# ryanelandt/PressureFieldContact.jl

Hardware: AMD Instinct MI355X
Metric: tet-tri clip+integrate ops/s (higher is better)
Workload: dtype f64

## Files before the change

pressurefieldcontact.jl_amd/csrc/pfc_hip.hip:

```cpp
#include "pfc_kernels.h"

#include <atomic>
#include <condition_variable>
#include <functional>
#include <mutex>
#include <thread>
#include <cmath>
#include <cstdlib>
#include <limits>
#include <cstdarg>
#include <cstdio>
#include <cstring>
#include <string>
#include <vector>

#include "../../include/pfc.h"
#include "pfc_sort.h"

namespace pfc {

__global__ void k_prep_tri(int n, const double *__restrict__ pt, const int *__restrict__ tri, TriRec *__restrict__ out) {
    int k = blockIdx.x * blockDim.x + threadIdx.x;
    if (k >= n) return;
    V3 a = ld3(pt + 3 * tri[3 * k]), b = ld3(pt + 3 * tri[3 * k + 1]), c = ld3(pt + 3 * tri[3 * k + 2]);
// ... 350 lines not shown
        hints[0].n = n; hints[0].sparse = sparse;
    }
    bool shape_is_sparse(int n) const {
        for (const ShapeHint &e : hints) if (e.n == n) return e.sparse;
        return false;
    }
    long long last_tslots = 0;
    Event ev[EV_COUNT];
    bool ev_valid = false;
    pfc_context *twin = nullptr;
    bool is_twin = false;
    DevBuf<int> fout;
    PinBuf<int> h_fout;
    int *fout_dev = nullptr;
    const int *fout_host = nullptr;
    int opt_fused = 1;
    int opt_fixed_order = 0;
    DevBuf<int> det;
    DevBuf<unsigned long long> sort_keys[2];
    DevBuf<int> canon_off, canon_fill, canon_item;
    int sort_tmp_items = 0;
    bool fixed_whole_list = false;
    DevBuf<char> sort_tmp;
    size_t sort_tmp_for = 0;
    int sort_tmp_bits = 0;
    int max_elem1 = 1, max_elem2 = 1;
    DevBuf<double> fx_rec, vfx_rec;
    DevBuf<int> vfx_head;
    DevBuf<int> fx_head;
    long long surv_sorted_serial = -1;
    size_t sort_cover = 0;
    size_t sort_cover_used = 0;
    int opt_vertex_fields = 1;
    int opt_clip_queue = 1;
    int fused_skip = 0;
    int fused_seq = 0;
    int fu_nw = 1;
    int last_fu_nw = 0, last_team = 0;
    int n_cu = 0;
    int opt_team = 48;
    DevBuf<unsigned long long> team;
    DevBuf<int> emit_ctr;
    PinBuf<int> h_emit;
    PinBuf<unsigned> h_more;
    bool fu_emit = false;
    int dual_fused_skip = 0;
    const double *fu_dpose = nullptr, *fu_dtwist = nullptr;
    double *fu_dwrench = nullptr, *fu_dsdot = nullptr;
    int fu_ndir = 0;
    bool pending_fused = false, last_fused = false;
    int opt_split_min = 1025;
    int opt_clip_min = 384;
    int opt_poison = 0;
    int split_n0 = 0;
    bool in_split = false;
    int last_parts = 1;
    Event ev_fork, ev_join, ev_join0;
    int twin_queue_fallback = 0;
    DevBuf<long long> surf_cnt, surf_off, surf_out;
    DevBuf<double> surf_part;
    DevBuf<int> surf_seg, surf_canon_off, surf_canon_fill, surf_canon_item;
    DevBuf<double> ljac_seed;
    DevBuf<double> ljac_out;
    DevBuf<double> ljac_io;
    DevBuf<int> ljac_ids;
    DevBuf<unsigned long long> surf_keys[2];
// ... 161 lines not shown
    double *d = h->trac_d.p;
    t.item = h->trac_item.p;
    t.nx = d; t.ny = d + n; t.nz = d + 2 * n; t.rx = d + 3 * n; t.ry = d + 4 * n; t.rz = d + 5 * n;
    t.dA = d + 6 * n; t.p = d + 7 * n;
    return t;
}

int eff_levels(const pfc_context *h) {
    return (h->opt_max_levels > 0 && h->opt_max_levels < h->max_levels) ? h->opt_max_levels : h->max_levels;
}

constexpr int kDualSelectMin = 512;
constexpr int kBpSmallBlockMin = 3072;

int bfs_levels_for(const pfc_context *h, int n_items, int levels) {
    int L = 0;
    if (h->opt_bfs_levels >= 0) {
        L = h->opt_bfs_levels;
    } else {
        const bool big = h->max_leaves >= 8192, mid = h->max_leaves >= 1024;
        const int n_eff = h->in_split ? 2 * n_items : n_items;
        const double target = big ? (n_eff >= 600 ? 1.0 : (n_eff >= 256 ? 1024.0 : (n_eff >= 128 ? 2048.0 : (n_eff >= 32 ? 16384.0 : 49152.0))))
                                  : (mid ? 256.0 : 64.0);
        double seeds = (double)n_items;
        while (seeds < target && L < 9) { seeds *= 4.0; ++L; }
    }
    return L > levels ? levels : L;
}

bool pile_mode(const pfc_context *h, int n_items) {
    return h->max_leaves < 8192 && n_items >= 1024 && n_items < kBpSmallBlockMin && h->shape_is_sparse(n_items) && !h->is_twin;
}

int bp_block_for(const pfc_context *h, int n_items) {
    if (n_items >= kBpSmallBlockMin) return 128;
    if (h->in_split) return 256;
    if (h->max_leaves >= 8192 && n_items >= 8 && n_items < 1024) return 512;
    if (pile_mode(h, n_items)) return 512;
    return 256;
}

void launch_broadphase(pfc_context *h, int n_items, int L, int *ccount, int *fcount, int *next_seed, int *ucount, hipStream_t st) {
    for (int lv = 0; lv < L; ++lv) {
        BpArgs b;
        b.items = h->items.p; b.fin = h->frontier[lv & 1].p; b.fout = h->frontier[(lv + 1) & 1].p;
        b.cand = h->cand.p; b.fcount = fcount; b.ccount = ccount; b.icnt = h->icnt.p; b.status = h->status.p;
        b.level = lv; b.fcap = (int)h->fcap; b.ccap = (int)h->ccap; b.n_items = n_items;
        double ub = (double)n_items * std::pow(4.0, (double)(lv < 15 ? lv : 15));
        size_t bound = ub > (double)h->fcap ? h->fcap : (size_t)ub;
        hipLaunchKernelGGL(k_bp_expand, dim3(grid_for(bound, 256, 2048)), dim3(256), 0, st, b);
    }
    {
        double ub = (double)n_items * std::pow(4.0, (double)(L < 15 ? L : 15));
        size_t bound = ub > (double)h->fcap ? h->fcap : (size_t)ub;
        DfsArgs d;
        d.items = h->items.p; d.cand = h->cand.p; d.ccount = ccount; d.ccap = (int)h->ccap; d.icnt = h->icnt.p;
        d.status = h->status.p; d.reserve = 3 * h->max_levels + 3; d.stamps = h->stamps.p; d.n_items = n_items;
        if (h->opt_no_filter) {
            d.seeds = h->frontier[L & 1].p; d.n_seed = fcount + L; d.seed_cap = (int)h->fcap; d.next_seed = next_seed;
            d.no_filter = 1;
            hipLaunchKernelGGL(k_bp_dfs, dim3(grid_for(bound, 1, 256 * 8)), dim3(64), 0, st, d);
        } else {
            Dfs32Args f;
            f.items = h->items.p; f.seeds = h->frontier[L & 1].p; f.n_seed = fcount + L; f.next_seed = next_seed;
            f.seed_cap = (int)h->fcap; f.cand = h->cand.p; f.ccount = ccount; f.ccap = (int)h->ccap;
            f.ucount = ucount; f.icnt = h->icnt.p; f.status = h->status.p; f.stamps = h->stamps.p;
// ... 57 lines not shown
    NpArgs np;
    np.items = h->items.p; np.cand = h->cand.p; np.ccount = ccount; np.ccap = (int)h->ccap; np.acc = h->acc.p;
    np.icnt = h->icnt.p; np.n_items = n_items; np.clip_n = h->opt_debug ? h->clip_n.p : nullptr; np.trac = trac_view(h);
    np.tcount = tcount; np.tcap = (int)h->tcap; np.status = h->status.p; np.debug = h->opt_debug;
    np.stamps = h->stamps.p;
    np.rec = h->rec.p; np.rgn = h->rgn.p; np.rr_cap = (int)(h->rcap / kRgn);
    np.poly_item = h->poly_item.p; np.poly = h->poly.p; np.pcap = (int)poly_cap(h->ccap);
    np.pcnt = h->pcnt.p; np.chunk_switch = kNpChunkSwitch; np.poly_cand = h->want_surv ? h->poly_cand.p : nullptr;
    np.surv = h->want_surv ? h->surv.p : nullptr; np.scount = pcount + 1;
    const int np_grid = grid_for(h->ccap, kNpBlock, kNpMaxBlocks);
    const int np_mode = h->opt_debug ? 1 : ((h->opt_fixed_order || (h->opt_clip_min > 0 && n_items >= h->opt_clip_min)) ? 2 : 0);
    if (np_mode == 1) {
        if (h->any_tet_tet) hipLaunchKernelGGL((k_narrow<true, 1>), dim3(np_grid), dim3(kNpBlock), 0, st, np);
        else hipLaunchKernelGGL((k_narrow<false, 1>), dim3(np_grid), dim3(kNpBlock), 0, st, np);
    } else if (np_mode == 0) {
        if (h->any_tet_tet) hipLaunchKernelGGL((k_narrow<true, 0>), dim3(np_grid), dim3(kNpBlock), 0, st, np);
        else hipLaunchKernelGGL((k_narrow<false, 0>), dim3(np_grid), dim3(kNpBlock), 0, st, np);
    } else {
        if (h->opt_clip_queue && !h->any_tet_tet) {
            hipLaunchKernelGGL(k_clip_queue, dim3(np_grid), dim3(kNpBlock), 0, st, np);
        } else if (h->in_split || (n_items >= 640 && n_items < 1024)) {
            if (h->any_tet_tet) hipLaunchKernelGGL((k_narrow<true, 3>), dim3(np_grid), dim3(kNpBlock), 0, st, np);
            else hipLaunchKernelGGL((k_narrow<false, 3>), dim3(np_grid), dim3(kNpBlock), 0, st, np);
        } else {
            if (h->any_tet_tet) hipLaunchKernelGGL((k_narrow<true, 2>), dim3(np_grid), dim3(kNpBlock), 0, st, np);
            else hipLaunchKernelGGL((k_narrow<false, 2>), dim3(np_grid), dim3(kNpBlock), 0, st, np);
        }
        IntegArgs ig;
        ig.items = h->items.p; ig.n_items = n_items; ig.ccount = ccount; ig.ccap = (int)h->ccap; ig.chunk_switch = kNpChunkSwitch;
        ig.pcnt = h->pcnt.p; ig.poly_item = h->poly_item.p; ig.poly = h->poly.p; ig.pcap = np.pcap;
        ig.poly_cand = np.poly_cand; ig.surv = np.surv; ig.scount = np.scount; ig.acc = h->acc.p; ig.rec = h->rec.p;
        ig.rgn = h->rgn.p; ig.rr_cap = np.rr_cap; ig.icnt = h->icnt.p; ig.status = h->status.p;
        ig.det = h->opt_fixed_order ? h->det.p : nullptr;
        if (h->opt_fixed_order) hipLaunchKernelGGL(k_integ_fixed, dim3(grid_for(h->ccap, 64, kNpMaxBlocks)), dim3(64), 0, st, ig);
        else hipLaunchKernelGGL(k_integ, dim3(grid_for(h->ccap, 64, kNpMaxBlocks)), dim3(64), 0, st, ig);
    }
    if (prof) HIP_TRY(h, hipEventRecord(h->ev[EV_NP], st));

    BrArgs br;
    br.items = h->items.p; br.n_items = n_items; br.acc = h->acc.p; br.res = h->res.p; br.icnt = h->icnt.p;
    br.trac = trac_view(h); br.tcount = tcount; br.tcap = (int)h->tcap; br.wrench = d_wrench; br.sdot = d_sdot;
    br.counts = d_counts;
    br.ctr = h->ctr.p; br.n_ctr = levels + 12; br.status = h->status.p; br.tail = h->tail_dev ? h->tail_dev : h->tail.p;
    br.rgn = h->rgn.p; br.i_pcount = (levels + 9) & ~1;
    if (h->opt_fixed_order && np_mode == 2) {
        FixedArgs fx;
        fx.rec = h->rec.p; fx.det = h->det.p; fx.n_items = n_items; fx.n_slots = (int)(h->rcap / kRgn) * kRgn; fx.items = h->items.p;
        fx.acc = h->acc.p; fx.status = h->status.p;
        hipLaunchKernelGGL(k_shift_fixed, dim3(n_items), dim3(64), 0, st, fx);
    }
    if (h->any_bristle) {
        ShiftArgs sh;
        sh.rec = h->rec.p; sh.rgn = h->rgn.p; sh.rr_cap = (int)(h->rcap / kRgn); sh.acc = h->acc.p;
        if (!(h->opt_fixed_order && np_mode == 2)) hipLaunchKernelGGL(k_shift, dim3(grid_for(h->rcap, 64, 2048)), dim3(64), 0, st, sh);
        hipLaunchKernelGGL(k_eig, dim3(n_items), dim3(64), 0, st, br);
        FricArgs fr;
        fr.items = h->items.p; fr.poly_item = h->poly_item.p; fr.poly = h->poly.p; fr.ccount = ccount; fr.ccap = (int)h->ccap;
        fr.chunk_switch = kNpChunkSwitch; fr.pcnt = h->pcnt.p;
        fr.pcap = np.pcap; fr.res = h->res.p; fr.acc = h->acc.p;
        fr.n_items = n_items; fr.status = h->status.p;
        fr.sink = FixedSink{nullptr, nullptr, nullptr, 0, 0, 0, 0, 0, nullptr};
        if (h->opt_fixed_order && np_mode == 2) {
            const size_t n_pos = h->ccap / 64 + 1, cap = fixed_fric_cap(h->ccap, n_items);
            HIP_TRY(h, hipMemsetAsync(h->vfx_head.p, 0xFF, sizeof(int) * (size_t)n_items, st));
            HIP_TRY(h, hipMemsetAsync(h->vfx_head.p + n_items, 0, sizeof(int) * 2, st));
            fr.sink = FixedSink{h->vfx_rec.p, h->vfx_head.p + n_items, h->vfx_head.p, 0, 2, (int)n_pos, (int)(2 * n_pos), (int)cap, h->status.p};
        }
        const bool vertex_fields = h->opt_vertex_fields && !h->opt_debug;
// ... 752 lines not shown
    if (!h) return PFC_ERR_BAD_ARG;
    if (h->multi)
        return multi_eval_device(h, n_items, 0, d_ins_ids, d_pose, nullptr, d_twist, d_s, nullptr, nullptr, nullptr, d_wrench, d_sdot,
                                 nullptr, nullptr, d_counts, stream);
    { const int rc = check_eval_args(h, n_items, d_ins_ids, d_pose, d_twist, d_s, d_wrench, d_sdot); if (rc != PFC_OK) return rc; }
    if (n_items == 0) { h->pending = false; h->last_n_items = 0; return PFC_OK; }
    HIP_TRY(h, hipSetDevice(h->device));
    hipStream_t st = stream ? (hipStream_t)stream : h->stream;
    h->split_n0 = 0;
    h->pending_fused = false;
    end_kept_pass(h);
    h->pending_more = false;
    int team = fused_team(h, n_items);
    if (team > 1 && !team_acquire(h)) team = fused_ok(h, n_items) ? 1 : 0;
    if (team) {
        h->fu_nw = team;
        const int rc_t = enqueue_fused(h, n_items, d_ins_ids, d_pose, d_twist, d_s, d_wrench, d_sdot, d_counts, st);
        h->fu_nw = 1;
        if (rc_t != PFC_OK) team_release(h);
        return rc_t;
    }
    if (h->fused_skip > 0 && n_items <= kFusedMaxItems) --h->fused_skip;
    const bool split = h->opt_split_min > 0 && n_items >= h->opt_split_min && d_ins_ids && !h->opt_debug && !h->opt_fixed_order &&
                       !h->want_surv && !h->is_twin && !pile_mode(h, n_items);
    if (!split) return enqueue_eval(h, n_items, d_ins_ids, d_pose, d_twist, d_s, d_wrench, d_sdot, d_counts, st);
    int rc = make_twin(h);
    if (rc != PFC_OK) return rc;
    pfc_context *t = h->twin;
    t->opt_profile = h->opt_profile; t->opt_max_levels = h->opt_max_levels; t->opt_bfs_levels = h->opt_bfs_levels;
    t->opt_poison = h->opt_poison;
    if (t->opt_clip_min != h->opt_clip_min) { t->opt_clip_min = h->opt_clip_min; t->ghave[0] = t->ghave[1] = false; }
    if (t->opt_clip_queue != h->opt_clip_queue) { t->opt_clip_queue = h->opt_clip_queue; t->ghave[0] = t->ghave[1] = false; }
    if (t->opt_vertex_fields != h->opt_vertex_fields) { t->opt_vertex_fields = h->opt_vertex_fields; t->ghave[0] = t->ghave[1] = false; }
    t->opt_graph = h->opt_graph;
    if (t->opt_no_filter != h->opt_no_filter) { t->opt_no_filter = h->opt_no_filter; t->ghave[0] = t->ghave[1] = false; }
    const int n0 = n_items / 2, n1 = n_items - n0;
    hipStream_t s0 = h->stream;
    HIP_TRY(h, hipEventRecord(h->ev_fork, st));
    if (s0 != st) HIP_TRY(h, hipStreamWaitEvent(s0, h->ev_fork, 0));
    HIP_TRY(h, hipStreamWaitEvent(t->stream, h->ev_fork, 0));
    h->in_split = true; t->in_split = true;
    rc = enqueue_eval(h, n0, d_ins_ids, d_pose, d_twist, d_s, d_wrench, d_sdot, d_counts, s0);
    h->in_split = false;
    if (rc != PFC_OK) return rc;
    rc = enqueue_eval(t, n1, d_ins_ids + n0, d_pose + 24 * (size_t)n0, d_twist + 6 * (size_t)n0,
                      d_s ? d_s + 6 * (size_t)n0 : nullptr, d_wrench + 6 * (size_t)n0, d_sdot + 6 * (size_t)n0,
                      d_counts ? d_counts + 4 * (size_t)n0 : nullptr, t->stream);
    if (rc != PFC_OK) { h->err = t->err; return rc; }
    HIP_TRY(h, hipEventRecord(h->ev_join, t->stream));
    HIP_TRY(h, hipStreamWaitEvent(st, h->ev_join, 0));
    if (s0 != st) {
        HIP_TRY(h, hipEventRecord(h->ev_join0, s0));
        HIP_TRY(h, hipStreamWaitEvent(st, h->ev_join0, 0));
    }
    h->split_n0 = n0;
    return PFC_OK;
}

namespace {

struct SurfFricOut {
    const double *s;
    double *fric, *fric_summary, *stiff;
};

int surface_enqueue(pfc_context *h, int n_items, const int *d_ins_ids, const double *d_pose, const double *d_twist, long long cap_poly,
// ... 1216 lines not shown
    copy_out_dual((const double *)h->pin_out.p, nk, d_wrench, d_sdot);
    return PFC_OK;
}

int pfc_set_option(pfc_handle h, const char *name, long long value) {
    if (!h || !name) return PFC_ERR_BAD_ARG;
    if (h->multi) {
        if (!std::strcmp(name, "multi_min")) { h->multi->opt_min_items = value < 1 ? 1 : (int)value; h->multi->part_n = 0; return PFC_OK; }
        h->multi->dev_kept = false;
        for (pfc_context *c : h->multi->shard) {
            const int rc = on_shard(h, c, [&](pfc_context *c1) { return pfc_set_option(c1, name, value); });
            if (rc != PFC_OK) return rc;
        }
        return PFC_OK;
    }
    end_kept_pass(h);
    if (!std::strcmp(name, "debug")) h->opt_debug = value != 0;
    else if (!std::strcmp(name, "profile")) h->opt_profile = value != 0;
    else if (!std::strcmp(name, "max_levels")) {
        if (value < 0 || value > (1 << 20) || (h->finalized && value > h->max_levels))
            return fail(h, PFC_ERR_BAD_ARG, "max_levels must be 0 (automatic) or 1..%d (depth of the finalized trees + 1)", h->max_levels);
        h->opt_max_levels = (int)value; h->ghave[0] = h->ghave[1] = false; h->dghave = false;
    }
    else if (!std::strcmp(name, "bfs_levels")) h->opt_bfs_levels = (int)value;
    else if (!std::strcmp(name, "graph")) h->opt_graph = value != 0;
    else if (!std::strcmp(name, "split_min")) h->opt_split_min = (int)value;
    else if (!std::strcmp(name, "dual_reuse")) h->opt_dual_reuse = (int)value;
    else if (!std::strcmp(name, "clip_min")) { h->opt_clip_min = (int)value; h->ghave[0] = h->ghave[1] = false; h->dghave = false; }
    else if (!std::strcmp(name, "clip_queue")) { h->opt_clip_queue = (int)value; h->ghave[0] = h->ghave[1] = false; h->dghave = false; }
    else if (!std::strcmp(name, "vertex_fields")) {
        if (value != 0 && value != 1) return fail(h, PFC_ERR_BAD_ARG, "vertex_fields must be 0 (per-point k_fric) or 1 (per-corner fields)");
        h->opt_vertex_fields = (int)value; h->ghave[0] = h->ghave[1] = false; h->dghave = false;
    }
    else if (!std::strcmp(name, "poison")) h->opt_poison = value != 0;
    else if (!std::strcmp(name, "fused")) { h->opt_fused = value != 0; h->fused_skip = 0; }
    else if (!std::strcmp(name, "team")) h->opt_team = value < 0 ? 0 : (value > kTeamMaxWg ? kTeamMaxWg : (int)value);
    else if (!std::strcmp(name, "team_fault")) h->opt_team_fault = (int)value;
    else if (!std::strcmp(name, "fused_f32")) h->opt_fused_f32 = value != 0;
    else if (!std::strcmp(name, "dual_fold")) { h->opt_dual_fold = value != 0; h->dghave = false; }
    else if (!std::strcmp(name, "fixed_order")) {
        const int on = value != 0;
        if (on != h->opt_fixed_order) {
            h->opt_fixed_order = on; h->fused_skip = 0;
            h->ghave[0] = h->ghave[1] = false; h->dghave = false;
            h->rec.release();
        }
    }
    else if (!std::strcmp(name, "no_filter")) { h->opt_no_filter = (int)value; h->ghave[0] = h->ghave[1] = false; h->dghave = false; }
    else return fail(h, PFC_ERR_BAD_ARG, "unknown option %s", name);
    return PFC_OK;
}

int pfc_get_stats(pfc_handle h, long long *out8) {
    if (!h || !out8) return PFC_ERR_BAD_ARG;
    if (h->multi) { for (int k = 0; k < 8; ++k) out8[k] = h->multi->stats[k]; return PFC_OK; }
    for (int k = 0; k < 8; ++k) out8[k] = h->stats[k];
    return PFC_OK;
}

int pfc_get_stage_ms(pfc_handle h, float *out6) {
    if (!h || !out6) return PFC_ERR_BAD_ARG;
    if (h->multi)
        return on_first_shard(h, [&](pfc_context *c) { return pfc_get_stage_ms(c, out6); });
    if (!h->ev_valid) return fail(h, PFC_ERR_STATE, "profile option was off for the last evaluation");
    HIP_TRY(h, hipSetDevice(h->device));
    HIP_TRY(h, hipEventSynchronize(h->ev[EV_FIN]));
// ... 350 lines not shown
```

pressurefieldcontact.jl_amd/csrc/pfc_kernels.h:

```cpp
#pragma once
#include <hip/hip_runtime.h>

namespace pfc {

constexpr int kInternal = -9999;
constexpr int kWave = 64;

enum : unsigned {
    kStNonFinite = 1u,
    kStFrontierOvf = 2u,
    kStCandOvf = 4u,
    kStTracOvf = 8u,
    kStBadIns = 16u,
    kStAbort = 32u,
    kStRecOvf = 64u,
    kStPolyOvf = 128u,
    kStHole = 256u,
    kStFixedSpan = 2048u,
    kStFixedCover = 8192u,
    kStFixedBig = 16384u,
    kStFixedList = 4096u,
};

struct alignas(16) NodeRec {
// ... 334 lines not shown
};
__device__ __forceinline__ FanFields fan_fields(const PointParams &c) {
    FanFields f;
    f.er0 = c.er0; f.er1 = c.er1; f.er2 = c.er2; f.er3 = c.er3;
    const V3 e = mk3(c.er0, c.er1, c.er2);
    f.d0 = __builtin_fma(-c.chi, dot(e, c.vl), 1.0);
    f.dg = cross(e, c.w) * (-c.chi);
    f.nq = c.nq;
    if (c.nq == 1) { f.qa = 0.33333333333333331483; f.qd = 0.0; f.qw = 1.0; }
    else { f.qa = 0.16666666666666674068; f.qd = 0.66666666666666651864 - 0.16666666666666674068; f.qw = 0.33333333333333331483; }
    return f;
}
__device__ __forceinline__ double fan_field_a(const FanFields &f, const V3 &c) {
    return __builtin_fma(f.er2, c.z, __builtin_fma(f.er1, c.y, __builtin_fma(f.er0, c.x, f.er3)));
}
__device__ __forceinline__ double fan_field_d(const FanFields &f, const V3 &c) {
    return __builtin_fma(f.dg.z, c.z, __builtin_fma(f.dg.y, c.y, __builtin_fma(f.dg.x, c.x, f.d0)));
}
__device__ __forceinline__ double fan_linear_a(const FanFields &f, const V3 &r) {
    return __builtin_fma(f.er2, r.z, __builtin_fma(f.er1, r.y, f.er0 * r.x));
}
__device__ __forceinline__ double fan_linear_d(const FanFields &f, const V3 &r) {
    return __builtin_fma(f.dg.z, r.z, __builtin_fma(f.dg.y, r.y, f.dg.x * r.x));
}
__device__ __forceinline__ double fan_sum(const FanFields &f, double f1, double f2, double fc) { return __builtin_fma(f.qa, f1 + f2, fc); }
__device__ __forceinline__ V3 fan_sum(const FanFields &f, const V3 &f1, const V3 &f2, const V3 &fc) {
    return mk3(fan_sum(f, f1.x, f2.x, fc.x), fan_sum(f, f1.y, f2.y, fc.y), fan_sum(f, f1.z, f2.z, fc.z));
}
__device__ __forceinline__ double fan_at(const FanFields &f, double S, double corner) { return __builtin_fma(f.qd, corner, S); }
__device__ __forceinline__ V3 fan_at(const FanFields &f, const V3 &S, const V3 &corner) {
    return mk3(fan_at(f, S.x, corner.x), fan_at(f, S.y, corner.y), fan_at(f, S.z, corner.z));
}

__device__ __forceinline__ int sat15_f32_core(const float *ea, const float *eb, const float *t, const float *R, float E) {
    float aR[9];
#pragma unroll
    for (int k = 0; k < 9; ++k) aR[k] = __builtin_fabsf(R[k]);
    float dmax;
#define R_(i, j) R[(i) + 3 * (j)]
#define AR_(i, j) aR[(i) + 3 * (j)]
#define AXIS_(tl, rsum) dmax = __builtin_fmaxf(dmax, (tl) - (rsum))
    {
        const float rb = __builtin_fmaf(AR_(0, 2), eb[2], __builtin_fmaf(AR_(0, 1), eb[1], AR_(0, 0) * eb[0]));
        dmax = __builtin_fabsf(t[0]) - (ea[0] + rb);
    }
#pragma unroll
    for (int i = 1; i < 3; ++i) {
        const float rb = __builtin_fmaf(AR_(i, 2), eb[2], __builtin_fmaf(AR_(i, 1), eb[1], AR_(i, 0) * eb[0]));
        AXIS_(__builtin_fabsf(t[i]), ea[i] + rb);
    }
#pragma unroll
    for (int j = 0; j < 3; ++j) {
        const float tl = __builtin_fabsf(__builtin_fmaf(R_(2, j), t[2], __builtin_fmaf(R_(1, j), t[1], R_(0, j) * t[0])));
        const float ra = __builtin_fmaf(AR_(2, j), ea[2], __builtin_fmaf(AR_(1, j), ea[1], AR_(0, j) * ea[0]));
        AXIS_(tl, ra + eb[j]);
    }
    constexpr int i100[3] = {1, 0, 0}, i221[3] = {2, 2, 1};
#pragma unroll
    for (int j = 0; j < 3; ++j) {
        const float tl = __builtin_fabsf(__builtin_fmaf(t[2], R_(1, j), -(t[1] * R_(2, j))));
        const float ra = __builtin_fmaf(ea[1], AR_(2, j), ea[2] * AR_(1, j));
        const float rb = __builtin_fmaf(eb[i100[j]], AR_(0, i221[j]), eb[i221[j]] * AR_(0, i100[j]));
        AXIS_(tl, ra + rb);
    }
#pragma unroll
    for (int j = 0; j < 3; ++j) {
// ... 201 lines not shown
```

pressurefieldcontact.jl_amd/csrc/pfc_np.h:

```cpp
#pragma once

struct TracSoA {
    int *item;
    double *nx, *ny, *nz, *rx, *ry, *rz, *dA, *p;
};

struct NpArgs {
    const ItemRec *items;
    const WorkRec *cand;
    const int *ccount;
    int ccap;
    double *acc;
    double *rec;
    int *rgn;
    int rr_cap;
    int *pcnt;
    int chunk_switch;
    int *poly_cand;
    int *icnt;
    int n_items;
    int *clip_n;
    int *poly_item;
    double *poly;
    int pcap;
// ... 851 lines not shown
                    for (int i = 0; i < 4; ++i) QZ(e, k, i) = z[k][i];
                QX(e, 0) = nh_in.x; QX(e, 1) = nh_in.y; QX(e, 2) = nh_in.z;
                QX(e, 3) = __longlong_as_double((long long)(((unsigned long long)(unsigned)cw.b << 32) | (unsigned long long)(unsigned)cw.item));
                qpos[e] = (unsigned short)pos;
            }
            q += __popcll(sm);
            wave_lds_sync();
            if (q >= kNpBlock) dense_round();
        }
        if (q > 0) dense_round();
        if (lane == 0) g.pcnt[ch] = pc;
    }
#undef QZ
#undef QX
}

struct IntegArgs {
    const ItemRec *items;
    int n_items;
    const int *ccount;
    int ccap, chunk_switch;
    const int *pcnt;
    int *poly_item;
    const double *poly;
    int pcap;
    const int *poly_cand;
    int *surv, *scount;
    double *acc, *rec;
    int *rgn;
    int rr_cap;
    int *icnt;
    unsigned *status;
    int *det;
};

template <int N, int L>
__device__ __forceinline__ double lds_rows_total(const double *buf, int lane, int lane0) {
    constexpr int RS = 64 + L;
    static_assert(N * L <= 64 && (L == 1 || L == 2 || L == 4), "rows x lanes per row must fit the wave");
    double t = 0.0;
    const int row = lane / L, part = lane % L;
    if (row < N) {
        const double *r = buf + row * RS + part;
        double t0 = 0.0, t1 = 0.0, t2 = 0.0, t3 = 0.0;
#pragma unroll
        for (int j = 0; j < 64 / L; j += 8) {
            const double a0 = r[L * j], a1 = r[L * (j + 1)], a2 = r[L * (j + 2)], a3 = r[L * (j + 3)];
            const double a4 = r[L * (j + 4)], a5 = r[L * (j + 5)], a6 = r[L * (j + 6)], a7 = r[L * (j + 7)];
            t0 += a0; t1 += a1; t2 += a2; t3 += a3;
            t0 += a4; t1 += a5; t2 += a6; t3 += a7;
        }
        t = (t0 + t1) + (t2 + t3);
    }
#pragma unroll
    for (int m = 1; m < L; m <<= 1) t += __shfl_xor(t, m, 64);
    const int dst_row = lane - lane0;
    const double out = __shfl(t, (dst_row >= 0 && dst_row < N) ? dst_row * L : 0, 64);
    return (dst_row >= 0 && dst_row < N) ? out : 0.0;
}

template <bool DET>
__device__ __forceinline__ void integ_body(const IntegArgs &g, double *m27) {
    constexpr int RS = 66;
    const int lane = threadIdx.x;
    int n_c = *g.ccount;
    if (n_c > g.ccap) n_c = g.ccap;
    const int C = np_chunk(n_c, g.chunk_switch);
    const int n_chunk = (n_c + C - 1) / C;
    const size_t P = (size_t)g.pcap;
    for (int ch = blockIdx.x; ch < n_chunk; ch += gridDim.x) {
        int cnt = __builtin_amdgcn_readfirstlane(g.pcnt[ch]);
        if (cnt > C) cnt = C;
        int cur = -1, n_tr = 0;
        bool cur_reg = false;
        V3 c0 = mk3(0.0, 0.0, 0.0);
        double s10[10];
#pragma unroll
        for (int k = 0; k < 10; ++k) s10[k] = 0.0;
        auto flush = [&]() {
            if (cur < 0 || !__any(n_tr > 0)) return;
            double t10 = 0.0, Wt = 0.0, sx = 0.0, sy = 0.0, sz = 0.0;
#pragma unroll
            for (int k = 0; k < 10; ++k) {
                const double t = wave_total(s10[k], lane);
                if (lane == (DET ? kRecTen + k : k)) t10 = t;
                if (k == 6) Wt = t;
                if (k == 7) sx = t;
                if (k == 8) sy = t;
                if (k == 9) sz = t;
            }
            if constexpr (DET) {
                const bool mom = !cur_reg && Wt > 0.0;
                double mine = 0.0;
                if (mom) {
// ... 85 lines not shown
                pp.w = w; pp.vl = vl; pp.chi = chi; pp.Ebar = Ebar; pp.er0 = er0; pp.er1 = er1; pp.er2 = er2; pp.er3 = er3; pp.nq = nq;
                auto points = [&](auto &&body) {
                    for (int k = 0; k < n; ++k) {
                        const V3 v1 = v2;
                        v2 = vn;
                        if (k + 1 < n) vn = mk3(o[(13 + 3 * k) * P], o[(14 + 3 * k) * P], o[(15 + 3 * k) * P]);
                        ntl += fan_triangle_points(pp, v1, v2, cen, nh, body);
                    }
                };
                if (lane_reg) {
                    const double v_c = it->v_c, mu_s = it->mu_s, mu_d = it->mu_d;
                    points([&](const V3 &r, const V3 &rdot, double p, double dA) {
                        const double p_dA = p * dA;
                        const V3 vt = vec_sub_vec_proj(rdot, nh);
                        const double m2 = dot_fma(vt, vt);
                        V3 T;
                        if (m2 < v_c * v_c) {
                            T = vt * (-(mu_s / v_c));
                        } else {
                            double ri = __builtin_amdgcn_rsq(m2);
                            const double hm = 0.5 * m2;
                            ri = ri * __builtin_fma(-hm * ri, ri, 1.5);
                            ri = ri * __builtin_fma(-hm * ri, ri, 1.5);
                            const double mg = m2 * ri;
                            const double mu = clamped_piecewise(mg, 2 * v_c, 3 * v_c, mu_s, mu_d);
                            T = vt * (-(mu * ri));
                        }
                        const V3 tk = (nh + T) * p_dA;
                        const V3 ta = cross_fma(r, tk);
                        fs[0] += ta.x; fs[1] += ta.y; fs[2] += ta.z;
                        fs[3] += tk.x; fs[4] += tk.y; fs[5] += tk.z;
                    });
                } else {
                    points([&](const V3 &r, const V3 &, double p, double dA) {
                        const double p_dA = p * dA;
                        W += p_dA;
                        const V3 rc = r - cen;
                        const double wx = p_dA * rc.x, wy = p_dA * rc.y, wz = p_dA * rc.z;
                        wr1[0] += wx; wr1[1] += wy; wr1[2] += wz;
                        wrr[0] = __builtin_fma(wx, rc.x, wrr[0]); wrr[1] = __builtin_fma(wx, rc.y, wrr[1]);
                        wrr[2] = __builtin_fma(wx, rc.z, wrr[2]); wrr[3] = __builtin_fma(wy, rc.y, wrr[3]);
                        wrr[4] = __builtin_fma(wy, rc.z, wrr[4]); wrr[5] = __builtin_fma(wz, rc.z, wrr[5]);
                    });
                }
            }
            const bool contributed = ntl > 0;
            unsigned long long todo = __ballot(has);
            while (todo) {
                const int f = __builtin_ctzll(todo);
                const int run_item = __builtin_amdgcn_readlane(item, f);
                const bool in_run = has && item == run_item;
                todo &= ~__ballot(in_run);
                const bool reg = __builtin_amdgcn_readlane((int)lane_reg, f) != 0;
                if (run_item != cur) {
                    flush();
                    cur = run_item;
                    cur_reg = reg;
                    c0 = mk3(readlane_f64(cen.x, f), readlane_f64(cen.y, f), readlane_f64(cen.z, f));
                    n_tr = 0;
#pragma unroll
                    for (int k = 0; k < 10; ++k) s10[k] = 0.0;
                    if (!reg) {
#pragma unroll
                        for (int k = 0; k < 27; ++k) m27[k * RS + lane] = 0.0;
                    }
                }
                if (!in_run || !contributed) continue;
                n_tr += ntl;
                if (reg) {
#pragma unroll
                    for (int k = 0; k < 6; ++k) s10[k] += fs[k];
                } else {
                    const V3 Sr = mk3(wr1[0] + W * cen.x, wr1[1] + W * cen.y, wr1[2] + W * cen.z);
                    const V3 ta = cross(Sr, nh);
                    s10[0] += ta.x; s10[1] += ta.y; s10[2] += ta.z;
                    s10[3] += nh.x * W; s10[4] += nh.y * W; s10[5] += nh.z * W;
// ... 9 lines not shown
                    q[5] = wrr[5] + 2.0 * wr1[2] * d.z + W * d.z * d.z;
                    double *mc = m27 + lane;
#define M27_(k, v) mc[(k) * RS] += (v)
                    M27_(0, W * nh.x * nh.x); M27_(1, W * nh.x * nh.y); M27_(2, W * nh.x * nh.z);
                    M27_(3, W * nh.y * nh.y); M27_(4, W * nh.y * nh.z); M27_(5, W * nh.z * nh.z);
                    const V3 an = cross(m1, nh);
                    M27_(6, an.x * nh.x); M27_(7, an.y * nh.x); M27_(8, an.z * nh.x);
                    M27_(9, an.x * nh.y); M27_(10, an.y * nh.y); M27_(11, an.z * nh.y);
                    M27_(12, an.x * nh.z); M27_(13, an.y * nh.z); M27_(14, an.z * nh.z);
                    const V3 q0c = mk3(q[0], q[1], q[2]), q1c = mk3(q[1], q[3], q[4]), q2c = mk3(q[2], q[4], q[5]);
                    const V3 m0 = cross(nh, q0c), m1c = cross(nh, q1c), m2c = cross(nh, q2c);
                    const V3 r0 = cross(nh, mk3(m0.x, m1c.x, m2c.x)), r1 = cross(nh, mk3(m0.y, m1c.y, m2c.y));
                    const V3 r2 = cross(nh, mk3(m0.z, m1c.z, m2c.z));
                    M27_(15, r0.x); M27_(16, r0.y); M27_(17, r0.z); M27_(18, r1.y); M27_(19, r1.z); M27_(20, r2.z);
#pragma unroll
                    for (int k = 0; k < 6; ++k) M27_(21 + k, q[k]);
#undef M27_
                }
            }
            if (has && (!contributed || lane_reg)) g.poly_item[idx] = 0;
            if (g.surv != nullptr) {
                const unsigned long long sm = __ballot(has);
                if (sm) {
                    int sbase = 0;
                    if (lane == 0) sbase = atomicAdd(g.scount, __popcll(sm));
                    sbase = __builtin_amdgcn_readfirstlane(sbase);
                    if (has) g.surv[sbase + __popcll(sm & ((1ull << lane) - 1ull))] = contributed ? g.poly_cand[idx] : -1;
                }
            }
        }
        flush();
    }
}
__global__ void __launch_bounds__(64, 2) k_integ(IntegArgs g) {
    __shared__ double m27[27 * 66];
    integ_body<false>(g, m27);
}
__global__ void __launch_bounds__(64, 2) k_integ_fixed(IntegArgs g) {
    __shared__ double m27[27 * 66];
    integ_body<true>(g, m27);
}

struct FricArgs {
    const ItemRec *items;
    const int *poly_item;
    const double *poly;
    const int *ccount;
    int ccap, chunk_switch;
    const int *pcnt;
    int pcap;
    int n_items;
    unsigned *status;
    const double *res;
    double *acc;
    FixedSink sink;
};
template <bool FX, bool VF>
__device__ __forceinline__ void fric_body(const FricArgs &g) {
    const int lane = threadIdx.x;
    const size_t P = (size_t)g.pcap;
    int n_c = *g.ccount;
    if (n_c > g.ccap) n_c = g.ccap;
    const int C = np_chunk(n_c, g.chunk_switch);
    const int n_chunk = (n_c + C - 1) / C;
    for (int ch = blockIdx.x; ch < n_chunk; ch += gridDim.x) {
      int cnt = __builtin_amdgcn_readfirstlane(g.pcnt[ch]);
      if (cnt > C) cnt = C;
      for (int p0 = 0; p0 < cnt; p0 += 64) {
        const int idx = ch * C + p0 + lane;
        const bool active = p0 + lane < cnt;
        double sum[6];
#pragma unroll
        for (int k = 0; k < 6; ++k) sum[k] = 0.0;
// ... 119 lines not shown
```

Before: 4.080 billion.

## Evaluate integration quadrature via per-corner linear fields with tolerance fallback

Adds a per-corner field path to the integration kernel. Pressure and distance at each fan quadrature point are obtained by linear combination of corner values rather than recomputed per point. A rounding-tolerance classifier decides whether each point is clearly inside or outside, and any undecided point falls back to the original per-point loop. The path is on by default for the non-fixed-order kernel, and a new option selects between modes. It adds a templated kernel variant and extra register pressure, and risks paying twice when the fallback triggers.

Result: slower. 3.763 billion (-7.8%).

```diff
diff --git a/pressurefieldcontact.jl_amd/csrc/pfc_hip.hip b/pressurefieldcontact.jl_amd/csrc/pfc_hip.hip
--- a/pressurefieldcontact.jl_amd/csrc/pfc_hip.hip
+++ b/pressurefieldcontact.jl_amd/csrc/pfc_hip.hip
@@ -406,6 +406,7 @@
     size_t sort_cover = 0;
     size_t sort_cover_used = 0;
     int opt_vertex_fields = 1;
+    int opt_integ_fields = -1;
     int opt_clip_queue = 1;
     int fused_skip = 0;
     int fused_seq = 0;
@@ -633,6 +634,10 @@
     return h->max_leaves < 8192 && n_items >= 1024 && n_items < kBpSmallBlockMin && h->shape_is_sparse(n_items) && !h->is_twin;
 }
 
+int integ_fields_of(const pfc_context *h) {
+    return h->opt_integ_fields >= 0 ? h->opt_integ_fields : (h->opt_fixed_order ? 0 : 1);
+}
+
 int bp_block_for(const pfc_context *h, int n_items) {
     if (n_items >= kBpSmallBlockMin) return 128;
     if (h->in_split) return 256;
@@ -756,8 +761,14 @@
         ig.poly_cand = np.poly_cand; ig.surv = np.surv; ig.scount = np.scount; ig.acc = h->acc.p; ig.rec = h->rec.p;
         ig.rgn = h->rgn.p; ig.rr_cap = np.rr_cap; ig.icnt = h->icnt.p; ig.status = h->status.p;
         ig.det = h->opt_fixed_order ? h->det.p : nullptr;
-        if (h->opt_fixed_order) hipLaunchKernelGGL(k_integ_fixed, dim3(grid_for(h->ccap, 64, kNpMaxBlocks)), dim3(64), 0, st, ig);
-        else hipLaunchKernelGGL(k_integ, dim3(grid_for(h->ccap, 64, kNpMaxBlocks)), dim3(64), 0, st, ig);
+        const int integ_fields = integ_fields_of(h);
+        ig.all_undecided = integ_fields == 2;
+        const dim3 ig_grid(grid_for(h->ccap, 64, kNpMaxBlocks));
+        if (h->opt_fixed_order) {
+            if (integ_fields) hipLaunchKernelGGL(k_integ_fixed<true>, ig_grid, dim3(64), 0, st, ig);
+            else hipLaunchKernelGGL(k_integ_fixed<false>, ig_grid, dim3(64), 0, st, ig);
+        } else if (integ_fields) hipLaunchKernelGGL(k_integ<true>, ig_grid, dim3(64), 0, st, ig);
+        else hipLaunchKernelGGL(k_integ<false>, ig_grid, dim3(64), 0, st, ig);
     }
     if (prof) HIP_TRY(h, hipEventRecord(h->ev[EV_NP], st));
 
@@ -1576,6 +1587,7 @@
     if (t->opt_clip_min != h->opt_clip_min) { t->opt_clip_min = h->opt_clip_min; t->ghave[0] = t->ghave[1] = false; }
     if (t->opt_clip_queue != h->opt_clip_queue) { t->opt_clip_queue = h->opt_clip_queue; t->ghave[0] = t->ghave[1] = false; }
     if (t->opt_vertex_fields != h->opt_vertex_fields) { t->opt_vertex_fields = h->opt_vertex_fields; t->ghave[0] = t->ghave[1] = false; }
+    if (t->opt_integ_fields != h->opt_integ_fields) { t->opt_integ_fields = h->opt_integ_fields; t->ghave[0] = t->ghave[1] = false; }
     t->opt_graph = h->opt_graph;
     if (t->opt_no_filter != h->opt_no_filter) { t->opt_no_filter = h->opt_no_filter; t->ghave[0] = t->ghave[1] = false; }
     const int n0 = n_items / 2, n1 = n_items - n0;
@@ -2858,6 +2870,10 @@
         if (value != 0 && value != 1) return fail(h, PFC_ERR_BAD_ARG, "vertex_fields must be 0 (per-point k_fric) or 1 (per-corner fields)");
         h->opt_vertex_fields = (int)value; h->ghave[0] = h->ghave[1] = false; h->dghave = false;
     }
+    else if (!std::strcmp(name, "integ_fields")) {
+        if (value < 0 || value > 2) return fail(h, PFC_ERR_BAD_ARG, "integ_fields must be 0 (per-point k_integ), 1 (per-corner fields) or 2 (per-corner kernel, every polygon redone per point)");
+        h->opt_integ_fields = (int)value; h->ghave[0] = h->ghave[1] = false; h->dghave = false;
+    }
     else if (!std::strcmp(name, "poison")) h->opt_poison = value != 0;
     else if (!std::strcmp(name, "fused")) { h->opt_fused = value != 0; h->fused_skip = 0; }
     else if (!std::strcmp(name, "team")) h->opt_team = value < 0 ? 0 : (value > kTeamMaxWg ? kTeamMaxWg : (int)value);
diff --git a/pressurefieldcontact.jl_amd/csrc/pfc_kernels.h b/pressurefieldcontact.jl_amd/csrc/pfc_kernels.h
--- a/pressurefieldcontact.jl_amd/csrc/pfc_kernels.h
+++ b/pressurefieldcontact.jl_amd/csrc/pfc_kernels.h
@@ -390,6 +390,32 @@
     return mk3(fan_at(f, S.x, corner.x), fan_at(f, S.y, corner.y), fan_at(f, S.z, corner.z));
 }
 
+struct FanTol {
+    double a, d;
+    bool ok;
+};
+__device__ __forceinline__ FanTol fan_tolerances(const PointParams &c, double X, double Y, double Z) {
+    const double e0 = __builtin_fabs(c.er0), e1 = __builtin_fabs(c.er1), e2 = __builtin_fabs(c.er2), e3 = __builtin_fabs(c.er3);
+    const double wx = __builtin_fabs(c.w.x), wy = __builtin_fabs(c.w.y), wz = __builtin_fabs(c.w.z);
+    const double vx = __builtin_fabs(c.vl.x), vy = __builtin_fabs(c.vl.y), vz = __builtin_fabs(c.vl.z);
+    const double ch = __builtin_fabs(c.chi);
+    const double Ma = ((e0 * X + e1 * Y) + e2 * Z) + e3;
+    const double B = ((e0 * (vx + (wy * Z + wz * Y)) + e1 * (vy + (wz * X + wx * Z))) + e2 * (vz + (wx * Y + wy * X)));
+    const double Md = 1.0 + ch * B;
+    const double big = 0x1p100, k = 128.0 * 0x1p-53;
+    FanTol t;
+    t.a = __builtin_fma(k, Ma, 0x1p-700);
+    t.d = k * Md;
+    t.ok = e0 <= big && e1 <= big && e2 <= big && e3 <= big && wx <= big && wy <= big && wz <= big && vx <= big && vy <= big &&
+           vz <= big && ch <= big && X <= big && Y <= big && Z <= big && 0.0 < c.Ebar && c.Ebar <= 0x1.fffffffffffffp1023;
+    return t;
+}
+__device__ __forceinline__ int fan_classify(const FanTol &t, double a, double d, double aE) {
+    if (a > t.a && d > t.d && aE > 0x1p-900 && aE <= 0x1.fffffffffffffp1023) return 1;
+    if (a < -t.a || d < -t.d) return 0;
+    return -1;
+}
+
 __device__ __forceinline__ int sat15_f32_core(const float *ea, const float *eb, const float *t, const float *R, float E) {
     float aR[9];
 #pragma unroll
diff --git a/pressurefieldcontact.jl_amd/csrc/pfc_np.h b/pressurefieldcontact.jl_amd/csrc/pfc_np.h
--- a/pressurefieldcontact.jl_amd/csrc/pfc_np.h
+++ b/pressurefieldcontact.jl_amd/csrc/pfc_np.h
@@ -907,6 +907,7 @@
     int *icnt;
     unsigned *status;
     int *det;
+    int all_undecided;
 };
 
 template <int N, int L>
@@ -934,7 +935,7 @@
     return (dst_row >= 0 && dst_row < N) ? out : 0.0;
 }
 
-template <bool DET>
+template <bool DET, bool VF>
 __device__ __forceinline__ void integ_body(const IntegArgs &g, double *m27) {
     constexpr int RS = 66;
     const int lane = threadIdx.x;
@@ -1086,16 +1087,73 @@
                         fs[3] += tk.x; fs[4] += tk.y; fs[5] += tk.z;
                     });
                 } else {
-                    points([&](const V3 &r, const V3 &, double p, double dA) {
-                        const double p_dA = p * dA;
+                    auto add = [&](double p_dA, const V3 &rc) {
                         W += p_dA;
-                        const V3 rc = r - cen;
                         const double wx = p_dA * rc.x, wy = p_dA * rc.y, wz = p_dA * rc.z;
                         wr1[0] += wx; wr1[1] += wy; wr1[2] += wz;
                         wrr[0] = __builtin_fma(wx, rc.x, wrr[0]); wrr[1] = __builtin_fma(wx, rc.y, wrr[1]);
                         wrr[2] = __builtin_fma(wx, rc.z, wrr[2]); wrr[3] = __builtin_fma(wy, rc.y, wrr[3]);
                         wrr[4] = __builtin_fma(wy, rc.z, wrr[4]); wrr[5] = __builtin_fma(wz, rc.z, wrr[5]);
-                    });
+                    };
+                    bool per_point = !VF;
+                    if constexpr (VF) {
+                        const FanFields ff = fan_fields(pp);
+                        const double a_c = fan_field_a(ff, cen), d_c = fan_field_d(ff, cen);
+                        struct Corner { V3 c, r; double a, d; };
+                        double X = __builtin_fabs(cen.x), Y = __builtin_fabs(cen.y), Z = __builtin_fabs(cen.z);
+                        auto corner = [&](const V3 &c) {
+                            Corner f;
+                            f.c = c; f.r = c - cen;
+                            f.a = fan_linear_a(ff, f.r); f.d = fan_linear_d(ff, f.r);
+                            return f;
+                        };
+                        X = fmax(X, fmax(__builtin_fabs(v2.x), __builtin_fabs(vn.x)));
+                        Y = fmax(Y, fmax(__builtin_fabs(v2.y), __builtin_fabs(vn.y)));
+                        Z = fmax(Z, fmax(__builtin_fabs(v2.z), __builtin_fabs(vn.z)));
+                        for (int k = 1; k + 1 < n; ++k) {
+                            X = fmax(X, __builtin_fabs(o[(10 + 3 * k) * P]));
+                            Y = fmax(Y, __builtin_fabs(o[(11 + 3 * k) * P]));
+                            Z = fmax(Z, __builtin_fabs(o[(12 + 3 * k) * P]));
+                        }
+                        const FanTol tol = fan_tolerances(pp, X, Y, Z);
+                        bool undecided = g.all_undecided != 0 || !tol.ok;
+                        Corner f2 = corner(v2);
+                        for (int k = 0; k < n; ++k) {
+                            const Corner f1 = f2;
+                            f2 = corner(vn);
+                            if (k + 1 < n) vn = mk3(o[(13 + 3 * k) * P], o[(14 + 3 * k) * P], o[(15 + 3 * k) * P]);
+                            const double area = triangle_area(f1.c, f2.c, cen, nh);
+                            if (!(0.0 < area)) continue;
+                            const double dA = ff.qw * area;
+                            const double Sa = fan_sum(ff, f1.a, f2.a, a_c), Sd = fan_sum(ff, f1.d, f2.d, d_c);
+                            const V3 Sx = fan_sum(ff, f1.r, f2.r, mk3(0.0, 0.0, 0.0));
+                            auto point = [&](double a, double d, const V3 &rc) {
+                                const double aE = a * Ebar;
+                                const int cls = fan_classify(tol, a, d, aE);
+                                if (cls < 0) undecided = true;
+                                if (cls <= 0) return;
+                                ++ntl;
+                                add((aE * d) * dA, rc);
+                            };
+                            auto at = [&](const Corner &q) { point(fan_at(ff, Sa, q.a), fan_at(ff, Sd, q.d), fan_at(ff, Sx, q.r)); };
+                            at(f2);
+                            if (ff.nq != 1) { at(f1); point(Sa, Sd, Sx); }
+                        }
+                        if (undecided) {
+                            per_point = true;
+                            ntl = 0;
+                            W = 0.0;
+#pragma unroll
+                            for (int k = 0; k < 3; ++k) wr1[k] = 0.0;
+#pragma unroll
+                            for (int k = 0; k < 6; ++k) wrr[k] = 0.0;
+                            v2 = mk3(o[(10 + 3 * (n - 1)) * P], o[(11 + 3 * (n - 1)) * P], o[(12 + 3 * (n - 1)) * P]);
+                            vn = mk3(o[10 * P], o[11 * P], o[12 * P]);
+                        }
+                    }
+                    if (per_point) {
+                        points([&](const V3 &r, const V3 &, double p, double dA) { add(p * dA, r - cen); });
+                    }
                 }
             }
             const bool contributed = ntl > 0;
@@ -1171,13 +1229,13 @@
         flush();
     }
 }
-__global__ void __launch_bounds__(64, 2) k_integ(IntegArgs g) {
+template <bool VF> __global__ void __launch_bounds__(64, 2) k_integ(IntegArgs g) {
     __shared__ double m27[27 * 66];
-    integ_body<false>(g, m27);
-}
-__global__ void __launch_bounds__(64, 2) k_integ_fixed(IntegArgs g) {
+    integ_body<false, VF>(g, m27);
+}
+template <bool VF> __global__ void __launch_bounds__(64, 2) k_integ_fixed(IntegArgs g) {
     __shared__ double m27[27 * 66];
-    integ_body<true>(g, m27);
+    integ_body<true, VF>(g, m27);
 }
 
 struct FricArgs {
```
